# lambdaclass/simpleworks

Measured on AMD Instinct MI355X. Metric: Marlin prove() constraints/sec at 2^20 R1CS; G1 MSM points/sec, higher is better.
Workload: dtype u32 limbs (384-bit Montgomery Fq for G1, 256-bit Fr); 1 GPU; marlin_prove: synthetic R1CS, 2^20 constraints = variables = non-zeros per matrix (|H| = |K| = 2^20), SRS + proving key device resident; per_gpu_units=1048576, multi_gpu=replicas (one proof per rank)

## Files before the change

### simpleworks_amd/_lib.py

```python
import ctypes
import json
import os

import numpy as np

_HERE = os.path.dirname(os.path.abspath(__file__))
LIB_PATH = os.environ.get("SWM_LIB_PATH") or os.path.join(_HERE, "libswmarlin.so")

_u64p = ctypes.POINTER(ctypes.c_uint64)
_u32p = ctypes.POINTER(ctypes.c_uint32)
_vp = ctypes.c_void_p
_sz = ctypes.c_size_t
_int = ctypes.c_int

ABI = {
    "swm_version": (_int, []),
    "swm_strerror": (ctypes.c_char_p, [_int]),
    "swm_init": (_int, [_int, ctypes.POINTER(_vp)]),
    "swm_destroy": (None, [_vp]),
    "swm_last_error": (ctypes.c_char_p, [_vp]),
    "swm_set_stream": (_int, [_vp, _vp]),
    "swm_set_msm_sharding": (_int, [_vp, ctypes.c_uint, ctypes.c_uint, _vp, _vp]),
    "swm_rccl_unique_id": (_int, [ctypes.c_void_p]),
    "swm_rccl_init": (_int, [_vp, ctypes.c_void_p, ctypes.c_uint, ctypes.c_uint]),
# ... 431 lines not shown
        return out

    def selftest_poly_eval_many(self, buf_mont, pieces, z_mont):
        buf = np.ascontiguousarray(buf_mont, dtype=np.uint64).reshape(-1, 4)
        pc = np.asarray(pieces, dtype=np.uint64).reshape(-1, 2)
        out = np.zeros((pc.shape[0], 4), dtype=np.uint64)
        self._poly(3, buf, buf.shape[0], 0, z_mont, pc, out)
        return out

    def selftest_ntt_from(self, src_mont, log_n, inverse=False, coset=False):
        src = np.ascontiguousarray(src_mont, dtype=np.uint64).reshape(-1, 4).copy()
        out = np.zeros((1 << log_n, 4), dtype=np.uint64)
        self._poly(4 + int(bool(inverse)) + 2 * int(bool(coset)), src, src.shape[0], log_n, None, None, out)
        return out, src

    def selftest_scan(self, words):
        w = np.ascontiguousarray(words, dtype=np.uint32).reshape(-1)
        out = np.zeros(w.size + 1, dtype=np.uint32)
        self._poly(8, w, w.size, 0, None, None, out)
        return out[:-1], int(out[-1])

    def selftest_sample_fr(self, rng, need):
        out = np.zeros((max(need, 1), 4), dtype=np.uint64)
        self._check(self.lib.swm_selftest_sample_fr(self.h, rng.h, need, _p64(out)), "swm_selftest_sample_fr")
        return out[:need]

    def selftest_mul_throughput(self, which, threads, iters):
        ms = ctypes.c_float(0)
        self._check(self.lib.swm_selftest_mul_throughput(self.h, which, threads, iters, ctypes.byref(ms)),
                    "swm_selftest_mul_throughput")
# ... 2 lines not shown
```

### simpleworks_amd/csrc/devops.cuh

```cuda
#pragma once
#include <chrono>
#include <exception>
#include <functional>
#include <utility>
#include <atomic>
#include "context.h"
#include "ff.cuh"
#include "fill.cuh"
#include "fr29.cuh"
#include "host/chacha.h"
#include "host/marlin_types.h"

namespace swm {

int ntt_run(swm_ctx* ctx, void* d_data, unsigned log_n, int inverse, int coset);
int ntt_run_from(swm_ctx* ctx, void* d_data, unsigned log_n, int inverse, int coset, const void* first_src, size_t src_len);
int ntt_sharded_run(swm_ctx* ctx, void* d_local, unsigned log_n, int inverse, int blocks_in);
struct SpmvPlanHost {
    uint64_t nnz = 0, max_row = 0;
    std::vector<uint32_t> chunks, lrows;
};
struct SpmvPlan {
    uint64_t nnz = 0, max_row = 0;
    const uint32_t* d_chunks = nullptr;
    const uint32_t* d_lrows = nullptr;
    uint32_t n_chunks = 0, n_lrows = 0;
};
void spmv_plan_build(const uint32_t* rowptr, size_t rows, SpmvPlanHost* plan);
int spmv_run(swm_ctx* ctx, const void* d_rowptr, const void* d_col, const void* d_val, const void* d_z, void* d_out,
             size_t rows, const SpmvPlan* plan = nullptr);
int batch_inverse_run(swm_ctx* ctx, void* d, size_t n);
// ... 847 lines not shown
```

### simpleworks_amd/csrc/marlin.hip

```cpp
#include <stdlib.h>
#include <string.h>
#include <unistd.h>
#include <algorithm>
#include <chrono>
#include <functional>
#include <memory>
#include "devops.cuh"
#include "g1.cuh"
#include "host/ahp.h"

#include "msm.h"
using namespace swm;

#define LAUNCHX(ctx, name, kernel, grid, block, shmem, ...)                         \
    do {                                                                            \
        prof_begin(ctx, name);                                                      \
        hipLaunchKernelGGL(kernel, grid, block, shmem, (ctx)->stream, __VA_ARGS__); \
        prof_end(ctx);                                                              \
        hip_check(ctx, hipGetLastError(), name);                                    \
    } while (0)

#include "host/pk_codec.h"
#include "host/host_handles.h"
struct swm_srs {
// ... 1012 lines not shown
    ew(ctx, "div_vh", 3 * part, [=] __device__(size_t j) {
        Fr acc = q[j + part];
        if (j + 2 * part < total) acc = fp_add(acc, q[j + 2 * part]);
        if (j + 3 * part < total) acc = fp_add(acc, q[j + 3 * part]);
        h[j] = acc;
        if (j < part) g[j] = fp_add(q[j], acc);
    });
}
void div_vk(swm_ctx* ctx, const Fr* q, size_t part, size_t total, Fr* h) {
    ew(ctx, "div_vk", 3 * part, [=] __device__(size_t j) {
        Fr acc = fp_zero<Fr>();
        for (uint64_t i = 1; j + i * part < total; i++) acc = fp_add(acc, q[j + i * part]);
        h[j] = acc;
    });
}
struct RAlphaNumerators {
    Fr n0, n1, n2, n3;
};
RAlphaNumerators r_alpha_numerators(const Fr& alpha, unsigned logH, uint64_t M) {
    Fr aH = alpha;
    for (unsigned i = 0; i < logH; i++) aH = fp_sqr(aH);
    Fr i4 = HDomain(M).gen;
    for (unsigned i = 0; i < logH; i++) i4 = fp_sqr(i4);
    return {fp_sub(aH, fp_one<Fr>()), fp_sub(aH, i4), fp_sub(aH, fp_sqr(i4)), fp_sub(aH, fp_mul(fp_sqr(i4), i4))};
}
struct IndexOnB {
    const Fr *ar, *ac, *arc, *av;
    const Fr *br, *bc, *brc, *bv;
    const Fr *cr, *cc, *crc, *cv;
};
// ... 24 lines not shown
    const std::vector<Fr> public_input;
    FiatShamirRng fs;
    VerifierState st;
    Fr rho_w, rho_a, rho_b;
    int lane = 0;
    LPoly P_w, P_za, P_zb, P_mask, P_t, P_g1, P_h1, P_g2, P_h2;
    LPoly idx_polys[12];
    std::map<std::string, LPoly*> polys;
    CommitJob j1[4], j2[3], j3[2];
    std::vector<Commitment> comms1 = std::vector<Commitment>(4), comms2 = std::vector<Commitment>(3),
                            comms3 = std::vector<Commitment>(2);
    bool mask_late = false;
    unsigned mask_pieces = 1;
    AsyncMsm mask_part[2];
    bool ra_closed_form = false;
    LcSet lcs;
    DVec mask, z, za_evals, zb_evals, za_loc, zb_loc, x_poly, x_evals, w_poly, za_poly, zb_poly, e_za, e_zb, e_z;
    DVec r_alpha_evals, e_ra, t_poly, q1, h1, g1x, f, h2;

    ProveState(const swm_pk& pk, ChaChaRng& rng, PhaseTrace& t, ProveShape shp, const ShardPlan& plan)
        : zk(rng), tr(t), shape(std::move(shp)), sp(plan), H(pk.H), K(pk.K), X(pk.X), Bsz(pk.B), M(4 * pk.H),
          logM(pk.logH + 2), nvars(pk.info.num_variables), ninst(shape.inst.size()), mask_len(3 * pk.H), dh(pk.H),
          public_input(shape.inst.begin() + 1, shape.inst.end()) {
        fs_init(fs, pk.vk, public_input);
        for (int m = 0; m < 3; m++) {
            const DVec* v[4] = {&pk.ar[m].row, &pk.ar[m].col, &pk.ar[m].val, &pk.ar[m].row_col};
            for (int j = 0; j < 4; j++) {
                idx_polys[4 * m + j].p = v[j]->p;
                idx_polys[4 * m + j].n = K;
                polys[kIndexerPolys[4 * m + j]] = &idx_polys[4 * m + j];
// ... 155 lines not shown
        sharded_interpolate_and_commit(ctx, pk, s, s.zb_loc, s.rho_b, s.zb_poly, &s.j1[2]);
    } else {
        rc_check(ctx, ntt_run_from(ctx, s.za_poly.p, pk.logH, 1, 0, s.za_evals.p, H));
        add_rho_vh(ctx, s.za_poly.p, H, s.rho_a);
        rc_check(ctx, ntt_run_from(ctx, s.zb_poly.p, pk.logH, 1, 0, s.zb_evals.p, H));
        add_rho_vh(ctx, s.zb_poly.p, H, s.rho_b);
        pc_commit_begin(ctx, pk, &s.lane, s.P_za.p, s.P_za.n, false, 0, true, &s.j1[1]);
        pc_commit_begin(ctx, pk, &s.lane, s.P_zb.p, s.P_zb.n, false, 0, true, &s.j1[2]);
    }
}

DVec on_mul_domain(swm_ctx* ctx, const ProveState& s, const Fr* coeffs, size_t n) {
    if (!s.sp.r2) return dv_ntt_from(ctx, coeffs, n, s.logM, false);
    return shard_evals(ctx, s.sp, coeffs, n, s.logM);
}
void round2_prework(swm_ctx* ctx, ProveState& s) {
    const uint64_t H = s.H, X = s.X;
    s.e_za = on_mul_domain(ctx, s, s.za_poly.p, H + 1);
    s.e_zb = on_mul_domain(ctx, s, s.zb_poly.p, H + 1);
    DVec z_poly = dv_zeros(ctx, H + 1);
    Fr* out = z_poly.p;
    const Fr* wc = s.P_w.p;
    const size_t w_len = s.P_w.n;
    const Fr* xp = s.x_poly.p;
    ew(ctx, "z_poly", H + 1, [=] __device__(size_t i) {
        Fr v = fp_zero<Fr>();
        if (i >= X && i - X < w_len) v = wc[i - X];
        if (i < w_len) v = fp_sub(v, wc[i]);
        if (i < X) v = fp_add(v, xp[i]);
        out[i] = v;
    });
    s.e_z = on_mul_domain(ctx, s, z_poly.p, H + 1);
}

void round1_commitments(swm_ctx* ctx, const swm_pk& pk, ProveState& s) {
    pc_commit_blind(pk, &s.j1[0], &s.zk, &s.P_w.rand);
    pc_commit_blind(pk, &s.j1[1], &s.zk, &s.P_za.rand);
    pc_commit_blind(pk, &s.j1[2], &s.zk, &s.P_zb.rand);
    pc_commit_blind(pk, &s.j1[3], nullptr, &s.P_mask.rand);
    if (s.mask_pieces > 1) {
        Fr c0 = s.mask.download(0, 1)[0];
        Fr c0s = fp_to_std(c0);
        G1XYZZ extra = g1_mul_limbs(pk.vk.vk.g, c0s.v, 8);
        for (unsigned k = 0; k + 1 < s.mask_pieces; k++) g1_add(extra, commit_wait(ctx, &s.mask_part[k]));
        s.j1[3].has_extra = true;
        s.j1[3].extra = extra;
    }
// ... 26 lines not shown
        s.e_ra = DVec(ctx, mloc);
        PowTable wt = root_pow_table(ctx, s.logM);
        Fr* out = s.e_ra.p;
        ew(ctx, "r_alpha_den", mloc, [=] __device__(size_t p) {
            const size_t i = mloc * (p / mblk) + s_rank * mblk + (p % mblk);
            out[p] = fp_sub(alpha, wt.at(i));
        });
        rc_check(ctx, batch_inverse_run(ctx, out, mloc));
        const RAlphaNumerators nu = r_alpha_numerators(alpha, pk.logH, M);
        ew(ctx, "r_alpha_scale", mloc, [=] __device__(size_t p) {
            const size_t i = mloc * (p / mblk) + s_rank * mblk + (p % mblk);
            const unsigned q = (unsigned)(i & 3);
            out[p] = fp_mul(out[p], q == 0 ? nu.n0 : q == 1 ? nu.n1 : q == 2 ? nu.n2 : nu.n3);
        });
        r_alpha_on_h(ctx, pk, s);
    } else {
        s.e_ra = DVec(ctx, M);
        PowTable wt = root_pow_table(ctx, s.logM);
        Fr* out = s.e_ra.p;
        ew(ctx, "r_alpha_den", M, [=] __device__(size_t i) { out[i] = fp_sub(alpha, wt.at(i)); });
        rc_check(ctx, batch_inverse_run(ctx, out, M));
        const RAlphaNumerators nu = r_alpha_numerators(alpha, pk.logH, M);
        Fr* rh = s.r_alpha_evals.p;
        ew(ctx, "r_alpha_scale", M, [=] __device__(size_t i) {
            const unsigned q = (unsigned)(i & 3);
            Fr v = fp_mul(out[i], q == 0 ? nu.n0 : q == 1 ? nu.n1 : q == 2 ? nu.n2 : nu.n3);
            out[i] = v;
            if (q == 0) rh[i >> 2] = v;
        });
    }
// ... 4 lines not shown
    const size_t nvars = s.nvars;
    const Fr eta_a = s.st.eta_a, eta_b = s.st.eta_b, eta_c = s.st.eta_c;
    s.t_poly = dv_zeros(ctx, H);
    {
        DVec ta(ctx, nvars), tb(ctx, nvars), tc(ctx, nvars);
        const Fr* ra = s.r_alpha_evals.p;
        rc_check(ctx, spmv_run(ctx, pk.at.rowptr.p, pk.at.col.p, pk.at.val.p, ra, ta.p, nvars, &pk.at.plan));
        rc_check(ctx, spmv_run(ctx, pk.bt.rowptr.p, pk.bt.col.p, pk.bt.val.p, ra, tb.p, nvars, &pk.bt.plan));
        rc_check(ctx, spmv_run(ctx, pk.ct.rowptr.p, pk.ct.col.p, pk.ct.val.p, ra, tc.p, nvars, &pk.ct.plan));
        Fr* out = s.t_poly.p;
        const Fr *pa = ta.p, *pb = tb.p, *pc = tc.p;
        ew(ctx, "t_evals", nvars, [=] __device__(size_t c) {
            Fr v = fp_add(fp_add(fp_mul(eta_a, pa[c]), fp_mul(eta_b, pb[c])), fp_mul(eta_c, pc[c]));
            out[reindex_by_subdomain(H, X, c)] = v;
        });
        dv_ntt(ctx, s.t_poly, pk.logH, true);
    }
    s.tr.tick("r2: t polynomial enqueued");
    s.P_t.p = s.t_poly.p;
    s.P_t.n = H;
    pc_commit_begin(ctx, pk, &s.lane, s.P_t.p, s.P_t.n, false, 0, false, &s.j2[0]);
}

void round2_q1(swm_ctx* ctx, const swm_pk& pk, ProveState& s) {
    const uint64_t H = s.H, M = s.M;
    const size_t Mloc = s.sp.Mloc;
    const Fr eta_a = s.st.eta_a, eta_b = s.st.eta_b, eta_c = s.st.eta_c;
    s.q1 = DVec(ctx, Mloc);
    {
        if (!s.ra_closed_form) {
            DVec ra_poly = dv_ntt_from(ctx, s.r_alpha_evals.p, H, pk.logH, true);
            s.e_ra = on_mul_domain(ctx, s, ra_poly.p, H);
        }
        DVec e_t = on_mul_domain(ctx, s, s.t_poly.p, H);
        Fr* out = s.q1.p;
        const Fr *pra = s.e_ra.p, *pza = s.e_za.p, *pzb = s.e_zb.p, *pt = e_t.p, *pz = s.e_z.p;
        ew(ctx, "round2_pointwise", Mloc, [=] __device__(size_t i) {
            Fr a = pza[i], b = pzb[i];
            Fr summed = fp_add(fp_add(fp_mul(eta_c, fp_mul(a, b)), fp_mul(eta_a, a)), fp_mul(eta_b, b));
// ... 47 lines not shown
    pc_commit_blind(pk, &s.j2[1], &s.zk, &s.P_g1.rand);
    pc_commit_blind(pk, &s.j2[2], nullptr, &s.P_h1.rand);
    commit_gather(ctx, {&s.j2[0].plain, &s.j2[1].plain, &s.j2[1].shifted, &s.j2[2].plain});
    pc_commit_end_round(ctx, pk, {&s.j2[0], &s.j2[1], &s.j2[2]}, {nullptr, &s.zk, nullptr},
                        {&s.P_t.rand, &s.P_g1.rand, &s.P_h1.rand}, s.comms2.data());
    if (unsat && !ctx->emulated_exchange)
        throw MarlinError(SWM_ERR_UNSATISFIED, "outer sumcheck does not hold: constraint system is not satisfied");
}

void round3_polys(swm_ctx* ctx, const swm_pk& pk, ProveState& s) {
    const uint64_t K = s.K, Bsz = s.Bsz;
    const Fr alpha = s.st.alpha, beta = s.st.beta;
    const Fr eta_a = s.st.eta_a, eta_b = s.st.eta_b, eta_c = s.st.eta_c;
    const Fr vhab = fp_mul(s.dh.vanishing(alpha), s.dh.vanishing(beta));
    s.f = DVec(ctx, K);
    {
        DVec inv(ctx, 3 * K);
        for (int m = 0; m < 3; m++) {
            Fr* out = inv.p + (size_t)m * K;
            const Fr *rk = pk.ar[m].row_K.p, *ck = pk.ar[m].col_K.p;
            ew(ctx, "round3_den_K", K, [=] __device__(size_t i) { out[i] = fp_mul(fp_sub(beta, rk[i]), fp_sub(alpha, ck[i])); });
        }
        rc_check(ctx, batch_inverse_run(ctx, inv.p, 3 * K));
        Fr* out = s.f.p;
        const Fr *ia = inv.p, *ib = inv.p + K, *ic = inv.p + 2 * K;
        const Fr *va = pk.ar[0].val_K.p, *vb = pk.ar[1].val_K.p, *vc = pk.ar[2].val_K.p;
        ew(ctx, "round3_f_K", K, [=] __device__(size_t i) {
            Fr t = fp_add(fp_add(fp_mul(fp_mul(eta_a, va[i]), ia[i]), fp_mul(fp_mul(eta_b, vb[i]), ib[i])),
                          fp_mul(fp_mul(eta_c, vc[i]), ic[i]));
            out[i] = fp_mul(vhab, t);
        });
        dv_ntt(ctx, s.f, pk.logK, true);
    }
    s.P_g2.p = s.f.p + 1; s.P_g2.n = K - 1; s.P_g2.has_bound = true; s.P_g2.bound = K - 2;
    pc_commit_begin(ctx, pk, &s.lane, s.P_g2.p, s.P_g2.n, true, K - 2, false, &s.j3[0]);
    s.h2 = DVec(ctx, 3 * K);
    const IndexOnB ix{pk.ar[0].row_B.p, pk.ar[0].col_B.p, pk.ar[0].row_col_B.p, pk.ar[0].val_B.p,
                      pk.ar[1].row_B.p, pk.ar[1].col_B.p, pk.ar[1].row_col_B.p, pk.ar[1].val_B.p,
                      pk.ar[2].row_B.p, pk.ar[2].col_B.p, pk.ar[2].row_col_B.p, pk.ar[2].val_B.p};
    const Round3Challenges ch{alpha, beta, fp_mul(beta, alpha), eta_a, eta_b, eta_c, vhab};
    if (s.sp.r3) {
        const size_t Bloc = Bsz / s.sp.SG, Bblk = Bloc / s.sp.SG, Kl = K / s.sp.SG, s_rank = s.sp.rank;
        DVec e_f = shard_evals(ctx, s.sp, s.f.p, K, pk.logB);
        DVec ab(ctx, Bloc);
        Fr* out = ab.p;
        const Fr* pf = e_f.p;
        ew(ctx, "round3_pointwise_B", Bloc, [=] __device__(size_t p) {
            const size_t i = Bloc * (p / Bblk) + s_rank * Bblk + (p % Bblk);
            out[p] = round3_a_minus_bf(ix, ch, i, pf[p]);
        });
        rc_check(ctx, ntt_sharded_run(ctx, ab.p, pk.logB, 1, 1));
        DVec loc(ctx, 3 * Kl);
        div_vk(ctx, ab.p, Kl, Bloc, loc.p);
        shard_gather_cyclic(ctx, loc.p, 3 * Kl, s.sp.slog_g, s.h2.p, 3 * K);
    } else {
        DVec e_f = dv_ntt_from(ctx, s.f.p, K, pk.logB, false);
        DVec ab(ctx, Bsz);
        Fr* out = ab.p;
        const Fr* pf = e_f.p;
        ew(ctx, "round3_pointwise_B", Bsz, [=] __device__(size_t i) { out[i] = round3_a_minus_bf(ix, ch, i, pf[i]); });
        dv_ntt(ctx, ab, pk.logB, true);
        div_vk(ctx, ab.p, K, Bsz, s.h2.p);
    }
    s.P_h2.p = s.h2.p;
    s.P_h2.n = 3 * K >= 3 ? 3 * K - 3 : 0;
}

std::vector<Fr> evaluations(swm_ctx* ctx, const swm_pk& pk, ProveState& s) {
    std::map<std::pair<std::string, bool>, Fr> eval_cache;
// ... 688 lines not shown
static void selftest_poly_impl(swm_ctx* ctx, int op, void* data, size_t n, size_t m, const uint64_t* z, const uint64_t* pieces,
                               size_t npieces, void* out) {
    Fr zz = fp_zero<Fr>();
    if (z) memcpy(zz.v, z, 32);
    if (op == 8) {
        DBuf<uint32_t> in(ctx, n), res(ctx, n);
        if (n) in.upload((const uint32_t*)data, n);
        const uint32_t total = scan_exclusive_u32(ctx, in.p, res.p, n);
        std::vector<uint32_t> h = res.download(0, n);
        if (n) memcpy(out, h.data(), n * 4);
        ((uint32_t*)out)[n] = total;
        return;
    }
    DVec a(ctx, n);
    if (n) a.upload((const Fr*)data, n);
    if (op == 0) {
        suffix_recurrence(ctx, a.p, n, m, zz);
        std::vector<Fr> h = a.download(0, n);
        if (n) memcpy(data, h.data(), n * sizeof(Fr));
    } else if (op == 1) {
        DivResult r = div_linear(ctx, a.p, n, zz);
        std::vector<Fr> h = r.work.download(0, n);
        if (n) memcpy(out, h.data(), n * sizeof(Fr));
    } else if (op == 2) {
        const Fr v = poly_eval(ctx, a.p, n, zz);
        memcpy(out, v.v, sizeof(Fr));
    } else if (op == 3) {
        for (size_t i = 0; i < npieces; i++)
            if (pieces[2 * i] > n || pieces[2 * i + 1] > n - pieces[2 * i]) throw MarlinError(SWM_ERR_INVALID_ARG, "piece out of range");
        DVec res(ctx, npieces);
// ... 1 lines not shown
        for (size_t i = 0; i < npieces; i++) items.push_back({a.p + pieces[2 * i], (size_t)pieces[2 * i + 1], res.p + i});
        EvalPoint ep = eval_point(ctx, zz);
        poly_eval_many(ctx, items, ep);
        std::vector<Fr> h = res.download(0, npieces);
        if (npieces) memcpy(out, h.data(), npieces * sizeof(Fr));
    } else {
        DVec t = dv_ntt_from(ctx, a.p, n, (unsigned)m, ((op - 4) & 1) != 0, ((op - 4) & 2) != 0);
        std::vector<Fr> h = t.download(0, t.n);
        memcpy(out, h.data(), t.n * sizeof(Fr));
        std::vector<Fr> s = a.download(0, n);
        if (n) memcpy(data, s.data(), n * sizeof(Fr));
    }
}
int swm_selftest_poly(swm_ctx* ctx, int op, void* data, size_t n, size_t m, const uint64_t z[4], const uint64_t* pieces,
                      size_t npieces, void* out) {
    if (!ctx || op < 0 || op > 8 || (n && !data)) return SWM_ERR_INVALID_ARG;
    if ((op >= 1 && op <= 3 && !z) || (op == 0 && (!z || m == 0)) || (op != 0 && !out) || (op == 3 && npieces && !pieces))
        return SWM_ERR_INVALID_ARG;
    if (op >= 4 && op <= 7 && (m < 1 || m > 28 || n > ((size_t)1 << m))) return SWM_ERR_INVALID_ARG;
    SWM_ON_DEVICE(ctx);
    SWM_GUARD(ctx, selftest_poly_impl(ctx, op, data, n, m, z, pieces, npieces, out));
}
static void selftest_sample_impl(swm_ctx* ctx, ChaChaRng& rng, size_t need, uint64_t* out_mont) {
    DVec d(ctx, need);
    sample_fr_bulk(ctx, rng, d.p, need);
    std::vector<Fr> h = d.download(0, need);
    if (need) memcpy(out_mont, h.data(), need * sizeof(Fr));
}
int swm_selftest_sample_fr(swm_ctx* ctx, swm_rng* rng, size_t need, uint64_t* out_mont) {
    if (!ctx || !rng || (need && !out_mont)) return SWM_ERR_INVALID_ARG;
    SWM_ON_DEVICE(ctx);
    SWM_GUARD(ctx, selftest_sample_impl(ctx, rng->r, need, out_mont));
}

// ... 41 lines not shown
```

### simpleworks_amd/csrc/ntt.hip

```cpp
#include <atomic>
#include "context.h"
#include "ff.cuh"
#include "fr29.cuh"
#include <string.h>
#include <algorithm>
#include <vector>

namespace swm {

static constexpr int NTT_THREADS = 256;
static constexpr unsigned NTT_MAX_LOG_R = 10;

struct NttPassArgs {
    const Fr* src;
    Fr* dst;
    unsigned log_n, log_r, log_ns;
    const Fr* tw_small;
    const Fr* tw_lo;
    const Fr* tw_hi;
    const Fr* cs_lo;
    const Fr* cs_hi;
    uint64_t src_len;
    const Fr* pass_tw;
    int coset_in;
    int scale_out;
    int coset_out;
    Fr n_inv;
};

__device__ __forceinline__ Fr two_level_pow(const Fr* lo, const Fr* hi, uint64_t e) {
    Fr a = lo[e & 1023];
    uint64_t h = e >> 10;
    if (h) a = fp_mul(a, hi[h]);
    return a;
}

__device__ __forceinline__ unsigned bitrev_u(unsigned x, unsigned bits) { return bits ? (__brev(x) >> (32 - bits)) : 0u; }

template <int J>
__global__ void __launch_bounds__(NTT_THREADS) ntt_pass(NttPassArgs a) {
    SWM_LIGHT_KERNEL();
    extern __shared__ __align__(16) unsigned char smem_raw[];
    Fr* tile = reinterpret_cast<Fr*>(smem_raw);
    const unsigned R = 1u << a.log_r;
    const uint64_t n = 1ull << a.log_n;
    const uint64_t stride = n >> a.log_r;
    const uint64_t j0 = (uint64_t)blockIdx.x * J;
    const uint64_t ns_mask = (1ull << a.log_ns) - 1;
    const unsigned tw_shift = a.log_n - a.log_ns - a.log_r;
    for (unsigned e0 = 0; e0 < R * J; e0 += 4 * NTT_THREADS) {
        Fr xs[4];
#pragma unroll
        for (int u = 0; u < 4; u++) {
            unsigned e = e0 + threadIdx.x + u * NTT_THREADS;
            if (e < R * J) {
                const uint64_t at = j0 + e % J + (uint64_t)(e / J) * stride;
                xs[u] = at < a.src_len ? a.src[at] : fp_zero<Fr>();
            }
        }
#pragma unroll
        for (int u = 0; u < 4; u++) {
            unsigned e = e0 + threadIdx.x + u * NTT_THREADS;
            if (e >= R * J) break;
            unsigned jj = e % J, t = e / J;
            uint64_t idx = j0 + jj + (uint64_t)t * stride;
            Fr x = xs[u];
            if (a.coset_in) x = fp_mul(x, two_level_pow(a.cs_lo, a.cs_hi, idx));
            if (a.log_ns != 0 && t != 0) {
                uint64_t k = (j0 + jj) & ns_mask;
                if (k) x = fp_mul(x, two_level_pow(a.tw_lo, a.tw_hi, (k * t) << tw_shift));
            }
            tile[t * J + jj] = x;
        }
    }
    __syncthreads();
    unsigned h = R >> 1;
    if (a.log_r & 1) {
        for (unsigned bq = threadIdx.x; bq < (R >> 1) * J; bq += NTT_THREADS) {
            unsigned jj = bq % J, pos = bq / J;
            unsigned i0 = pos, i1 = i0 + h;
            Fr u = tile[i0 * J + jj], v = tile[i1 * J + jj];
            tile[i0 * J + jj] = fp_add(u, v);
// ... 30 lines not shown
    for (unsigned e = threadIdx.x; e < R * J; e += NTT_THREADS) {
        unsigned jj, u;
        if (a.log_ns == 0) {
            u = e % R;
            jj = e / R;
        } else {
            jj = e % J;
            u = e / J;
        }
        uint64_t j = j0 + jj;
        uint64_t k = j & ns_mask;
        uint64_t o = ((j - k) << a.log_r) + k + ((uint64_t)u << a.log_ns);
        Fr x = tile[bitrev_u(u, a.log_r) * J + jj];
        if (a.scale_out) {
            Fr s = a.n_inv;
            if (a.coset_out) s = fp_mul(s, two_level_pow(a.cs_lo, a.cs_hi, o));
            x = fp_mul(x, s);
        }
        a.dst[o] = x;
    }
}

struct LazyPlan {
    Spread29 r2;
    Spread29 s1[6];
    Spread29 s2[6];
    Spread29 s4;
    uint32_t reduce;
    uint32_t out_below_2r;
};
struct NttLazyArgs {
    NttPassArgs a;
    LazyPlan plan;
    int last_pass;
// ... 18 lines not shown
    return x;
}
template <int J>
__global__ void __launch_bounds__(NTT_THREADS, 4) ntt_pass_lazy(NttLazyArgs args) {
    SWM_LIGHT_KERNEL();
    extern __shared__ __align__(16) unsigned char smem_raw[];
    uint32_t* tile = reinterpret_cast<uint32_t*>(smem_raw);
    const NttPassArgs& a = args.a;
    const LazyPlan& P = args.plan;
    const unsigned R = 1u << a.log_r;
    const uint64_t n = 1ull << a.log_n;
    const uint64_t stride = n >> a.log_r;
    const uint64_t j0 = (uint64_t)blockIdx.x * J;
    const uint64_t ns_mask = (1ull << a.log_ns) - 1;
    const unsigned tw_shift = a.log_n - a.log_ns - a.log_r;
    for (unsigned e0 = 0; e0 < R * J; e0 += 4 * NTT_THREADS) {
        Fr xs[4];
#pragma unroll
        for (int u = 0; u < 4; u++) {
            unsigned e = e0 + threadIdx.x + u * NTT_THREADS;
            if (e < R * J) {
                const uint64_t at = j0 + e % J + (uint64_t)(e / J) * stride;
                xs[u] = at < a.src_len ? a.src[at] : fp_zero<Fr>();
            }
        }
#pragma unroll
        for (int u = 0; u < 4; u++) {
            unsigned e = e0 + threadIdx.x + u * NTT_THREADS;
            if (e >= R * J) break;
            unsigned jj = e % J, t = e / J;
            uint64_t idx = j0 + jj + (uint64_t)t * stride;
            Fr29 x = fr29_unpack(xs[u]);
            if (a.coset_in) x = fr29_mul_fenced(x, two_level_pow29(a.cs_lo, a.cs_hi, idx));
            if (a.log_ns != 0) {
                uint64_t k = (j0 + jj) & ns_mask;
                const Fr29 tw = a.pass_tw ? fr29_unpack(a.pass_tw[((uint64_t)t << a.log_ns) + k])
                                          : two_level_pow29(a.tw_lo, a.tw_hi, (k * t) << tw_shift);
                x = fr29_mul_fenced(x, tw);
            }
            tile_put(tile, t * J + jj, x);
        }
    }
    __syncthreads();
    unsigned h = R >> 1;
    if (a.log_r & 1) {
        for (unsigned bq = threadIdx.x; bq < (R >> 1) * J; bq += NTT_THREADS) {
            unsigned jj = bq % J, pos = bq / J;
            unsigned i0 = pos, i1 = i0 + h;
// ... 38 lines not shown
    for (unsigned e = threadIdx.x; e < R * J; e += NTT_THREADS) {
        unsigned jj, u;
        if (a.log_ns == 0) {
            u = e % R;
            jj = e / R;
        } else {
            jj = e % J;
            u = e / J;
        }
        uint64_t j = j0 + jj;
        uint64_t k = j & ns_mask;
        uint64_t o = ((j - k) << a.log_r) + k + ((uint64_t)u << a.log_ns);
        Fr29 x = tile_get(tile, bitrev_u(u, a.log_r) * J + jj);
        if (a.scale_out) {
            Fr29 sc = fr29_unpack(a.n_inv);
            if (a.coset_out) sc = fr29_mul_fenced(two_level_pow29(a.cs_lo, a.cs_hi, o), sc);
            x = fr29_canonical(fr29_mul_fenced(x, sc), true);
        } else if (args.last_pass) {
            x = fr29_canonical(x, P.out_below_2r != 0);
        }
        a.dst[o] = fr29_pack(x);
    }
}

static Fr host_root_of_unity(unsigned log_n, bool inverse) {
    Fr w;
    const uint32_t root[8] = SWM_FR_ROOT47_MONT;
    for (int i = 0; i < 8; i++) w.v[i] = root[i];
    for (unsigned i = log_n; i < 47; i++) w = fp_sqr(w);
    if (inverse) w = fp_inv(w);
    return w;
}

static int upload_powers(swm_ctx* ctx, const Fr& base, size_t count, void** out, bool lazy29 = false) {
    std::vector<Fr> h(count);
    Fr cur = lazy29 ? fp_from_u64<Fr>(32) : fp_one<Fr>();
// ... 124 lines not shown
        P.s1[st] = lazy_spread(2 * B, 1);
        P.s2[st] = lazy_spread(4 * B, 2);
        const bool red = 4 * B > 64 || st + 1 == nsteps;
        if (red) P.reduce |= 1u << st;
        B = red ? 4 : 4 * B;
    }
    P.s4 = lazy_spread(4, 1);
    P.out_below_2r = B <= 2 ? 1u : 0u;
    return P;
}

int ntt_run_from(swm_ctx* ctx, void* d_data, unsigned log_n, int inverse, int coset, const void* first_src, size_t src_len);
int ntt_run(swm_ctx* ctx, void* d_data, unsigned log_n, int inverse, int coset) {
    return ntt_run_from(ctx, d_data, log_n, inverse, coset, nullptr, 0);
}
int ntt_run_from(swm_ctx* ctx, void* d_data, unsigned log_n, int inverse, int coset, const void* first_src, size_t src_len) {
    if (log_n > 30) return set_err(ctx, SWM_ERR_INVALID_ARG, "ntt: log_n > 30 unsupported");
    const uint64_t n = 1ull << log_n;
    if (first_src && src_len > n) src_len = n;
    ctx->stat_ntt_calls++;
    ctx->log_call('n', log_n);
    ctx->stat_ntt_elems += n;
    Fr* data = reinterpret_cast<Fr*>(d_data);
    const unsigned maxr = NTT_MAX_LOG_R;
    static const bool lazy = env_switch("SWM_NTT_LAZY", 1, 0, 1) != 0;
    NttTables *rt = nullptr, *ct = nullptr;
    SWM_TRY(get_root_tables_form(ctx, log_n, inverse, lazy, &rt));
    if (coset) SWM_TRY(get_coset_tables(ctx, log_n, inverse, &ct, lazy));
    Fr n_inv = fp_one<Fr>();
    if (inverse) n_inv = fp_inv(fp_from_u64<Fr>(n));
    if (lazy) n_inv = fp_mul(n_inv, fp_from_u64<Fr>(32));
    unsigned npass = log_n <= maxr ? 1 : (log_n + maxr - 1) / maxr;
    unsigned radices[8];
    {
        unsigned rem = log_n;
        for (unsigned p = 0; p < npass; p++) {
            unsigned r = (rem + (npass - p) - 1) / (npass - p);
            radices[p] = r;
            rem -= r;
        }
    }
    Fr *tmp = nullptr, *tmp2 = nullptr;
    SWM_TRY(scratch(ctx, "ntt.tmp", n * sizeof(Fr), (void**)&tmp));
    if (npass % 2 == 1 && npass >= 3) SWM_TRY(scratch(ctx, "ntt.tmp2", n * sizeof(Fr), (void**)&tmp2));
    const Fr* src = first_src ? reinterpret_cast<const Fr*>(first_src) : data;
    if (npass == 1 && !first_src) {
        SWM_HIP(ctx, hipMemcpyAsync(tmp, data, n * sizeof(Fr), hipMemcpyDeviceToDevice, ctx->stream));
        src = tmp;
    }
    unsigned log_ns = 0;
    for (unsigned p = 0; p < npass; p++) {
        NttPassArgs a;
        a.src = src;
        if (p == npass - 1) a.dst = data;
        else if (tmp2) a.dst = (p % 2 == 0) ? tmp : tmp2;
        else a.dst = (src == tmp) ? data : tmp;
        a.src_len = (p == 0 && first_src) ? (uint64_t)src_len : n;
        a.log_n = log_n;
        a.log_r = radices[p];
        a.log_ns = log_ns;
        SWM_TRY(get_small_table(ctx, a.log_r, inverse, &a.tw_small, lazy));
        a.tw_lo = reinterpret_cast<const Fr*>(rt->lo);
        a.tw_hi = reinterpret_cast<const Fr*>(rt->hi);
        a.cs_lo = ct ? reinterpret_cast<const Fr*>(ct->lo) : nullptr;
        a.cs_hi = ct ? reinterpret_cast<const Fr*>(ct->hi) : nullptr;
        a.pass_tw = nullptr;
        if (lazy && log_ns != 0) SWM_TRY(get_pass_table(ctx, log_n, inverse, log_ns, a.log_r, rt, &a.pass_tw));
        a.coset_in = (coset && !inverse && p == 0) ? 1 : 0;
        a.scale_out = (inverse && p == npass - 1) ? 1 : 0;
        a.coset_out = (coset && inverse && p == npass - 1) ? 1 : 0;
        a.n_inv = n_inv;
        uint64_t cols = n >> a.log_r;
        if (lazy) {
            NttLazyArgs la;
            la.a = a;
            la.plan = lazy_plan(a.log_r, (p > 0 || a.coset_in) ? 2u : 1u);
            la.last_pass = p == npass - 1 ? 1 : 0;
            unsigned J = 1;
            if (npass > 1) {
                J = (log_n >= 19 ? 1024u : 512u) >> a.log_r;
                if (J < 1) J = 1;
                if (J > 16) J = 16;
                while (J > cols) J >>= 1;
            }
            const size_t elems = (size_t)J << a.log_r;
            size_t shmem = (elems + (elems >> 5) + 1) * 36;
            if (shmem < 64) shmem = 64;
            dim3 grid((unsigned)(cols / J)), block(NTT_THREADS);
            if (shmem > 64 * 1024) {
                static std::atomic<size_t> granted[64];
                if (J != 1 || shmem > 160 * 1024) return set_err(ctx, SWM_ERR_INVALID_ARG, "ntt: tile does not fit LDS");
                if (granted[ctx->device & 63].load() < shmem) {
                    SWM_HIP(ctx, hipFuncSetAttribute((const void*)ntt_pass_lazy<1>, hipFuncAttributeMaxDynamicSharedMemorySize, (int)shmem));
                    granted[ctx->device & 63].store(shmem);
                }
            }
            switch (J) {
                case 1: SWM_LAUNCH(ctx, "ntt_pass", ntt_pass_lazy<1>, grid, block, shmem, la); break;
                case 2: SWM_LAUNCH(ctx, "ntt_pass", ntt_pass_lazy<2>, grid, block, shmem, la); break;
                case 4: SWM_LAUNCH(ctx, "ntt_pass", ntt_pass_lazy<4>, grid, block, shmem, la); break;
                case 8: SWM_LAUNCH(ctx, "ntt_pass", ntt_pass_lazy<8>, grid, block, shmem, la); break;
                default: SWM_LAUNCH(ctx, "ntt_pass", ntt_pass_lazy<16>, grid, block, shmem, la); break;
            }
        } else if (npass == 1) {
            size_t shmem = sizeof(Fr) << a.log_r;
            if (shmem < 64) shmem = 64;
            SWM_LAUNCH(ctx, "ntt_pass", ntt_pass<1>, dim3((unsigned)cols), dim3(NTT_THREADS), shmem, a);
        } else {
            unsigned J = (log_n >= 19 ? 1024u : 512u) >> a.log_r;
            if (J < 1) J = 1;
            if (J > 16) J = 16;
            while (J > cols) J >>= 1;
            size_t shmem = (sizeof(Fr) * J) << a.log_r;
            dim3 grid((unsigned)(cols / J)), block(NTT_THREADS);
            switch (J) {
                case 1: SWM_LAUNCH(ctx, "ntt_pass", ntt_pass<1>, grid, block, shmem, a); break;
                case 2: SWM_LAUNCH(ctx, "ntt_pass", ntt_pass<2>, grid, block, shmem, a); break;
                case 4: SWM_LAUNCH(ctx, "ntt_pass", ntt_pass<4>, grid, block, shmem, a); break;
                case 8: SWM_LAUNCH(ctx, "ntt_pass", ntt_pass<8>, grid, block, shmem, a); break;
                default: SWM_LAUNCH(ctx, "ntt_pass", ntt_pass<16>, grid, block, shmem, a); break;
            }
        }
        log_ns += a.log_r;
        src = a.dst;
    }
    return SWM_OK;
}


// ... 72 lines not shown
```

Baseline: 22.04 million constraints/s.

## Evaluate Marlin round-2/3 quotients on size-H cosets instead of 4H domain

Round 2 now evaluates z_A, z_B, z and t on two cosets of H (plus the H domain itself) rather than running full 4H-size NTTs. Round 2 also does an inverse NTT per coset and recovers the three H-sized pieces with a small closed-form solve that uses the 4th root of unity and 1/2. Round 3 reuses the already-known evaluations of f on K and only transforms the three remaining cosets. Multi-coset NTTs are batched through blockIdx.y, with coset twiddles and folding of inputs longer than n done inside the pass kernels. The aim is to cut NTT size and memory traffic at the cost of added kernel-argument complexity and a new code path restricted to non-sharded runs.

```diff
diff --git a/simpleworks_amd/_lib.py b/simpleworks_amd/_lib.py
--- a/simpleworks_amd/_lib.py
+++ b/simpleworks_amd/_lib.py
@@ -469,6 +469,20 @@
         self._poly(4 + int(bool(inverse)) + 2 * int(bool(coset)), src, src.shape[0], log_n, None, None, out)
         return out, src
 
+    def selftest_ntt_cosets(self, coeffs_mont, log_n, ks):
+        src = np.ascontiguousarray(coeffs_mont, dtype=np.uint64).reshape(-1, 4).copy()
+        kk = np.ascontiguousarray(ks, dtype=np.uint64).reshape(-1)
+        out = np.zeros((kk.size << log_n, 4), dtype=np.uint64)
+        self._check(self.lib.swm_selftest_poly(self.h, 9, src.ctypes.data, src.shape[0], log_n, _p64(np.zeros(4, np.uint64)),
+                                               _p64(kk), kk.size, out.ctypes.data), "swm_selftest_poly")
+        return out.reshape(kk.size, 1 << log_n, 4)
+
+    def selftest_intt_cosets3(self, evals_mont, log_n):
+        ev = np.ascontiguousarray(evals_mont, dtype=np.uint64).reshape(-1, 4).copy()
+        out = np.zeros_like(ev)
+        self._poly(10, ev, ev.shape[0], log_n, None, None, out)
+        return out
+
     def selftest_scan(self, words):
         w = np.ascontiguousarray(words, dtype=np.uint32).reshape(-1)
         out = np.zeros(w.size + 1, dtype=np.uint32)
diff --git a/simpleworks_amd/csrc/devops.cuh b/simpleworks_amd/csrc/devops.cuh
--- a/simpleworks_amd/csrc/devops.cuh
+++ b/simpleworks_amd/csrc/devops.cuh
@@ -15,6 +15,8 @@
 
 int ntt_run(swm_ctx* ctx, void* d_data, unsigned log_n, int inverse, int coset);
 int ntt_run_from(swm_ctx* ctx, void* d_data, unsigned log_n, int inverse, int coset, const void* first_src, size_t src_len);
+int ntt_cosets_fwd(swm_ctx* ctx, const void* coeffs, size_t len, unsigned log_n, const unsigned* ks, unsigned ncos, void* out);
+int ntt_cosets_inv(swm_ctx* ctx, void* data, unsigned log_n, unsigned ncos);
 int ntt_sharded_run(swm_ctx* ctx, void* d_local, unsigned log_n, int inverse, int blocks_in);
 struct SpmvPlanHost {
     uint64_t nnz = 0, max_row = 0;
diff --git a/simpleworks_amd/csrc/marlin.hip b/simpleworks_amd/csrc/marlin.hip
--- a/simpleworks_amd/csrc/marlin.hip
+++ b/simpleworks_amd/csrc/marlin.hip
@@ -1050,6 +1050,20 @@
         h[j] = acc;
     });
 }
+#ifndef SWM_OUTER_COSETS
+#define SWM_OUTER_COSETS 1
+#endif
+static constexpr uint64_t OUTER_COSETS_MIN_H = 16;
+struct Cosets3 {
+    Fr p0, p1, p2;
+};
+__device__ __forceinline__ Cosets3 cosets3_solve(const Fr& u0, const Fr& u1, const Fr& u2, const Fr& iota, const Fr& half) {
+    const Fr p1 = fp_mul(fp_sub(u0, u2), half);
+    const Fr e = fp_mul(fp_add(u0, u2), half);
+    const Fr d = fp_sub(u1, fp_mul(iota, p1));
+    return {fp_mul(fp_add(e, d), half), p1, fp_mul(fp_sub(e, d), half)};
+}
+static Fr fr_half() { return fp_inv(fp_from_u64<Fr>(2)); }
 struct RAlphaNumerators {
     Fr n0, n1, n2, n3;
 };
@@ -1104,6 +1118,7 @@
     unsigned mask_pieces = 1;
     AsyncMsm mask_part[2];
     bool ra_closed_form = false;
+    bool cosets = false;
     LcSet lcs;
     DVec mask, z, za_evals, zb_evals, za_loc, zb_loc, x_poly, x_evals, w_poly, za_poly, zb_poly, e_za, e_zb, e_z;
     DVec r_alpha_evals, e_ra, t_poly, q1, h1, g1x, f, h2;
@@ -1289,10 +1304,19 @@
     if (!s.sp.r2) return dv_ntt_from(ctx, coeffs, n, s.logM, false);
     return shard_evals(ctx, s.sp, coeffs, n, s.logM);
 }
+DVec on_cosets12(swm_ctx* ctx, const ProveState& s, const Fr* coeffs, size_t n) {
+    static const unsigned ks[2] = {1, 2};
+    DVec v(ctx, 2 * s.H);
+    rc_check(ctx, ntt_cosets_fwd(ctx, coeffs, n, s.dh.log, ks, 2, v.p));
+    return v;
+}
 void round2_prework(swm_ctx* ctx, ProveState& s) {
     const uint64_t H = s.H, X = s.X;
-    s.e_za = on_mul_domain(ctx, s, s.za_poly.p, H + 1);
-    s.e_zb = on_mul_domain(ctx, s, s.zb_poly.p, H + 1);
+    s.cosets = SWM_OUTER_COSETS && !s.sp.r1 && !s.sp.r2 && H >= OUTER_COSETS_MIN_H && s.mask_len == 3 * H &&
+               !env_flag("SWM_RALPHA_TRANSFORMS");
+    auto on_domain = [&](const Fr* coeffs, size_t n) { return s.cosets ? on_cosets12(ctx, s, coeffs, n) : on_mul_domain(ctx, s, coeffs, n); };
+    s.e_za = on_domain(s.za_poly.p, H + 1);
+    s.e_zb = on_domain(s.zb_poly.p, H + 1);
     DVec z_poly = dv_zeros(ctx, H + 1);
     Fr* out = z_poly.p;
     const Fr* wc = s.P_w.p;
@@ -1305,7 +1329,7 @@
         if (i < X) v = fp_add(v, xp[i]);
         out[i] = v;
     });
-    s.e_z = on_mul_domain(ctx, s, z_poly.p, H + 1);
+    s.e_z = on_domain(z_poly.p, H + 1);
 }
 
 void round1_commitments(swm_ctx* ctx, const swm_pk& pk, ProveState& s) {
@@ -1362,6 +1386,22 @@
             out[p] = fp_mul(out[p], q == 0 ? nu.n0 : q == 1 ? nu.n1 : q == 2 ? nu.n2 : nu.n3);
         });
         r_alpha_on_h(ctx, pk, s);
+    } else if (s.cosets) {
+        const uint64_t H = s.H;
+        const unsigned logH = pk.logH;
+        s.e_ra = DVec(ctx, 3 * H);
+        PowTable wt = root_pow_table(ctx, s.logM);
+        Fr* out = s.e_ra.p;
+        ew(ctx, "r_alpha_den", 3 * H, [=] __device__(size_t p) { out[p] = fp_sub(alpha, wt.at(((p & (H - 1)) << 2) + (p >> logH))); });
+        rc_check(ctx, batch_inverse_run(ctx, out, 3 * H));
+        const RAlphaNumerators nu = r_alpha_numerators(alpha, pk.logH, M);
+        Fr* rh = s.r_alpha_evals.p;
+        ew(ctx, "r_alpha_scale", 3 * H, [=] __device__(size_t p) {
+            const size_t q = p >> logH;
+            Fr v = fp_mul(out[p], q == 0 ? nu.n0 : q == 1 ? nu.n1 : nu.n2);
+            out[p] = v;
+            if (q == 0) rh[p] = v;
+        });
     } else {
         s.e_ra = DVec(ctx, M);
         PowTable wt = root_pow_table(ctx, s.logM);
@@ -1396,6 +1436,23 @@
             Fr v = fp_add(fp_add(fp_mul(eta_a, pa[c]), fp_mul(eta_b, pb[c])), fp_mul(eta_c, pc[c]));
             out[reindex_by_subdomain(H, X, c)] = v;
         });
+        if (s.cosets) {
+            s.q1 = DVec(ctx, 3 * H);
+            Fr* q = s.q1.p;
+            const Fr *rh = s.r_alpha_evals.p, *za = s.za_evals.p, *zb = s.zb_evals.p, *th = s.t_poly.p, *zz = s.z.p, *xe = s.x_evals.p;
+            const uint64_t ratio = H / X;
+            const size_t nwit = s.shape.nwit, ninst = s.ninst;
+            ew(ctx, "round2_pointwise_h", H, [=] __device__(size_t k) {
+                Fr zk = xe[k];
+                if (k % ratio != 0) {
+                    const size_t wi = k - k / ratio - 1;
+                    zk = wi < nwit ? zz[ninst + wi] : fp_zero<Fr>();
+                }
+                const Fr a = za[k], b = zb[k];
+                const Fr summed = fp_add(fp_add(fp_mul(eta_c, fp_mul(a, b)), fp_mul(eta_a, a)), fp_mul(eta_b, b));
+                q[k] = fp_sub(fp_mul(rh[k], summed), fp_mul(zk, th[k]));
+            });
+        }
         dv_ntt(ctx, s.t_poly, pk.logH, true);
     }
     s.tr.tick("r2: t polynomial enqueued");
@@ -1404,7 +1461,47 @@
     pc_commit_begin(ctx, pk, &s.lane, s.P_t.p, s.P_t.n, false, 0, false, &s.j2[0]);
 }
 
+void round2_q1_cosets(swm_ctx* ctx, const swm_pk& pk, ProveState& s) {
+    const uint64_t H = s.H;
+    const Fr eta_a = s.st.eta_a, eta_b = s.st.eta_b, eta_c = s.st.eta_c;
+    if (!s.ra_closed_form) {
+        DVec ra_poly = dv_ntt_from(ctx, s.r_alpha_evals.p, H, pk.logH, true);
+        DVec e12 = on_cosets12(ctx, s, ra_poly.p, H);
+        s.e_ra = DVec(ctx, 3 * H);
+        hip_check(ctx, hipMemcpyAsync(s.e_ra.p + H, e12.p, 2 * H * sizeof(Fr), hipMemcpyDeviceToDevice, ctx->stream), "copy");
+    }
+    {
+        DVec e_t = on_cosets12(ctx, s, s.t_poly.p, H);
+        Fr* out = s.q1.p + H;
+        const Fr *pra = s.e_ra.p + H, *pza = s.e_za.p, *pzb = s.e_zb.p, *pt = e_t.p, *pz = s.e_z.p;
+        ew(ctx, "round2_pointwise", 2 * H, [=] __device__(size_t i) {
+            Fr a = pza[i], b = pzb[i];
+            Fr summed = fp_add(fp_add(fp_mul(eta_c, fp_mul(a, b)), fp_mul(eta_a, a)), fp_mul(eta_b, b));
+            out[i] = fp_sub(fp_mul(pra[i], summed), fp_mul(pz[i], pt[i]));
+        });
+        s.e_za.release();
+        s.e_zb.release();
+        s.e_z.release();
+    }
+    rc_check(ctx, ntt_cosets_inv(ctx, s.q1.p, pk.logH, 3));
+    s.h1 = DVec(ctx, 3 * H);
+    s.g1x = DVec(ctx, H);
+    const Fr* q = s.q1.p;
+    const Fr* mp = s.mask.p;
+    Fr *h = s.h1.p, *g = s.g1x.p;
+    const Fr iota = HDomain(4).gen, half = fr_half();
+    ew(ctx, "q1_cosets_solve_div_vh", H, [=] __device__(size_t j) {
+        const Cosets3 c = cosets3_solve(q[j], q[j + H], q[j + 2 * H], iota, half);
+        const Fr p0 = fp_add(c.p0, mp[j]), p1 = fp_add(c.p1, mp[j + H]), p2 = fp_add(c.p2, mp[j + 2 * H]);
+        const Fr hj = fp_add(p1, p2);
+        h[j] = hj;
+        h[j + H] = p2;
+        h[j + 2 * H] = fp_zero<Fr>();
+        g[j] = fp_add(p0, hj);
+    });
+}
 void round2_q1(swm_ctx* ctx, const swm_pk& pk, ProveState& s) {
+    if (s.cosets) return round2_q1_cosets(ctx, pk, s);
     const uint64_t H = s.H, M = s.M;
     const size_t Mloc = s.sp.Mloc;
     const Fr eta_a = s.st.eta_a, eta_b = s.st.eta_b, eta_c = s.st.eta_c;
@@ -1482,6 +1579,8 @@
     const Fr eta_a = s.st.eta_a, eta_b = s.st.eta_b, eta_c = s.st.eta_c;
     const Fr vhab = fp_mul(s.dh.vanishing(alpha), s.dh.vanishing(beta));
     s.f = DVec(ctx, K);
+    const bool f_cosets = SWM_OUTER_COSETS && !s.sp.r3 && Bsz == 4 * K && K >= OUTER_COSETS_MIN_H;
+    DVec f_K;
     {
         DVec inv(ctx, 3 * K);
         for (int m = 0; m < 3; m++) {
@@ -1493,12 +1592,17 @@
         Fr* out = s.f.p;
         const Fr *ia = inv.p, *ib = inv.p + K, *ic = inv.p + 2 * K;
         const Fr *va = pk.ar[0].val_K.p, *vb = pk.ar[1].val_K.p, *vc = pk.ar[2].val_K.p;
+        if (f_cosets) {
+            f_K = DVec(ctx, K);
+            out = f_K.p;
+        }
         ew(ctx, "round3_f_K", K, [=] __device__(size_t i) {
             Fr t = fp_add(fp_add(fp_mul(fp_mul(eta_a, va[i]), ia[i]), fp_mul(fp_mul(eta_b, vb[i]), ib[i])),
                           fp_mul(fp_mul(eta_c, vc[i]), ic[i]));
             out[i] = fp_mul(vhab, t);
         });
-        dv_ntt(ctx, s.f, pk.logK, true);
+        if (f_cosets) rc_check(ctx, ntt_run_from(ctx, s.f.p, pk.logK, 1, 0, f_K.p, K));
+        else dv_ntt(ctx, s.f, pk.logK, true);
     }
     s.P_g2.p = s.f.p + 1; s.P_g2.n = K - 1; s.P_g2.has_bound = true; s.P_g2.bound = K - 2;
     pc_commit_begin(ctx, pk, &s.lane, s.P_g2.p, s.P_g2.n, true, K - 2, false, &s.j3[0]);
@@ -1521,6 +1625,20 @@
         DVec loc(ctx, 3 * Kl);
         div_vk(ctx, ab.p, Kl, Bloc, loc.p);
         shard_gather_cyclic(ctx, loc.p, 3 * Kl, s.sp.slog_g, s.h2.p, 3 * K);
+    } else if (f_cosets) {
+        static const unsigned ks[3] = {1, 2, 3};
+        DVec e_f(ctx, 3 * K);
+        rc_check(ctx, ntt_cosets_fwd(ctx, s.f.p, K, pk.logK, ks, 3, e_f.p));
+        DVec ab(ctx, Bsz);
+        Fr* out = ab.p;
+        const Fr *pf = e_f.p, *fk = f_K.p;
+        const unsigned logK = pk.logK;
+        ew(ctx, "round3_pointwise_B", Bsz, [=] __device__(size_t i) {
+            const size_t k = i & 3, j = i >> 2;
+            out[i] = round3_a_minus_bf(ix, ch, i, k ? pf[((k - 1) << logK) + j] : fk[j]);
+        });
+        dv_ntt(ctx, ab, pk.logB, true);
+        div_vk(ctx, ab.p, K, Bsz, s.h2.p);
     } else {
         DVec e_f = dv_ntt_from(ctx, s.f.p, K, pk.logB, false);
         DVec ab(ctx, Bsz);
@@ -2239,6 +2357,32 @@
     }
     DVec a(ctx, n);
     if (n) a.upload((const Fr*)data, n);
+    if (op == 9) {
+        unsigned ks[4];
+        for (size_t c = 0; c < npieces; c++) ks[c] = (unsigned)pieces[c];
+        DVec t(ctx, npieces << m);
+        rc_check(ctx, ntt_cosets_fwd(ctx, a.p, n, (unsigned)m, ks, (unsigned)npieces, t.p));
+        std::vector<Fr> h = t.download(0, t.n);
+        memcpy(out, h.data(), t.n * sizeof(Fr));
+        return;
+    }
+    if (op == 10) {
+        const size_t N = (size_t)1 << m;
+        rc_check(ctx, ntt_cosets_inv(ctx, a.p, (unsigned)m, 3));
+        DVec t(ctx, 3 * N);
+        const Fr* u = a.p;
+        Fr* o = t.p;
+        const Fr iota = HDomain(4).gen, half = fr_half();
+        ew(ctx, "cosets3_solve", N, [=] __device__(size_t j) {
+            const Cosets3 c = cosets3_solve(u[j], u[j + N], u[j + 2 * N], iota, half);
+            o[j] = c.p0;
+            o[j + N] = c.p1;
+            o[j + 2 * N] = c.p2;
+        });
+        std::vector<Fr> h = t.download(0, t.n);
+        memcpy(out, h.data(), t.n * sizeof(Fr));
+        return;
+    }
     if (op == 0) {
         suffix_recurrence(ctx, a.p, n, m, zz);
         std::vector<Fr> h = a.download(0, n);
@@ -2270,10 +2414,16 @@
 }
 int swm_selftest_poly(swm_ctx* ctx, int op, void* data, size_t n, size_t m, const uint64_t z[4], const uint64_t* pieces,
                       size_t npieces, void* out) {
-    if (!ctx || op < 0 || op > 8 || (n && !data)) return SWM_ERR_INVALID_ARG;
+    if (!ctx || op < 0 || op > 10 || (n && !data)) return SWM_ERR_INVALID_ARG;
     if ((op >= 1 && op <= 3 && !z) || (op == 0 && (!z || m == 0)) || (op != 0 && !out) || (op == 3 && npieces && !pieces))
         return SWM_ERR_INVALID_ARG;
     if (op >= 4 && op <= 7 && (m < 1 || m > 28 || n > ((size_t)1 << m))) return SWM_ERR_INVALID_ARG;
+    if (op == 9) {
+        if (m < 1 || m > 26 || n > ((size_t)2 << m) || npieces < 1 || npieces > 4 || !pieces) return SWM_ERR_INVALID_ARG;
+        for (size_t c = 0; c < npieces; c++)
+            if (pieces[c] > 3) return SWM_ERR_INVALID_ARG;
+    }
+    if (op == 10 && (m < 1 || m > 26 || n != ((size_t)3 << m))) return SWM_ERR_INVALID_ARG;
     SWM_ON_DEVICE(ctx);
     SWM_GUARD(ctx, selftest_poly_impl(ctx, op, data, n, m, z, pieces, npieces, out));
 }
diff --git a/simpleworks_amd/csrc/ntt.hip b/simpleworks_amd/csrc/ntt.hip
--- a/simpleworks_amd/csrc/ntt.hip
+++ b/simpleworks_amd/csrc/ntt.hip
@@ -26,6 +26,10 @@
     int scale_out;
     int coset_out;
     Fr n_inv;
+    uint64_t src_cstride, dst_cstride;
+    uint32_t cos_k[4];
+    int fold_in;
+    Fr fold[4];
 };
 
 __device__ __forceinline__ Fr two_level_pow(const Fr* lo, const Fr* hi, uint64_t e) {
@@ -48,6 +52,9 @@
     const uint64_t j0 = (uint64_t)blockIdx.x * J;
     const uint64_t ns_mask = (1ull << a.log_ns) - 1;
     const unsigned tw_shift = a.log_n - a.log_ns - a.log_r;
+    const Fr* src = a.src + blockIdx.y * a.src_cstride;
+    Fr* dst = a.dst + blockIdx.y * a.dst_cstride;
+    const uint64_t cs_k = a.cos_k[blockIdx.y];
     for (unsigned e0 = 0; e0 < R * J; e0 += 4 * NTT_THREADS) {
         Fr xs[4];
 #pragma unroll
@@ -55,7 +62,8 @@
             unsigned e = e0 + threadIdx.x + u * NTT_THREADS;
             if (e < R * J) {
                 const uint64_t at = j0 + e % J + (uint64_t)(e / J) * stride;
-                xs[u] = at < a.src_len ? a.src[at] : fp_zero<Fr>();
+                xs[u] = at < a.src_len ? src[at] : fp_zero<Fr>();
+                if (a.fold_in && at + n < a.src_len) xs[u] = fp_add(xs[u], fp_mul(a.fold[blockIdx.y], src[at + n]));
             }
         }
 #pragma unroll
@@ -65,7 +73,7 @@
             unsigned jj = e % J, t = e / J;
             uint64_t idx = j0 + jj + (uint64_t)t * stride;
             Fr x = xs[u];
-            if (a.coset_in) x = fp_mul(x, two_level_pow(a.cs_lo, a.cs_hi, idx));
+            if (a.coset_in) x = fp_mul(x, two_level_pow(a.cs_lo, a.cs_hi, idx * cs_k));
             if (a.log_ns != 0 && t != 0) {
                 uint64_t k = (j0 + jj) & ns_mask;
                 if (k) x = fp_mul(x, two_level_pow(a.tw_lo, a.tw_hi, (k * t) << tw_shift));
@@ -126,10 +134,10 @@
         Fr x = tile[bitrev_u(u, a.log_r) * J + jj];
         if (a.scale_out) {
             Fr s = a.n_inv;
-            if (a.coset_out) s = fp_mul(s, two_level_pow(a.cs_lo, a.cs_hi, o));
+            if (a.coset_out) s = fp_mul(s, two_level_pow(a.cs_lo, a.cs_hi, o * cs_k));
             x = fp_mul(x, s);
         }
-        a.dst[o] = x;
+        dst[o] = x;
     }
 }
 
@@ -178,6 +186,9 @@
     const uint64_t j0 = (uint64_t)blockIdx.x * J;
     const uint64_t ns_mask = (1ull << a.log_ns) - 1;
     const unsigned tw_shift = a.log_n - a.log_ns - a.log_r;
+    const Fr* src = a.src + blockIdx.y * a.src_cstride;
+    Fr* dst = a.dst + blockIdx.y * a.dst_cstride;
+    const uint64_t cs_k = a.cos_k[blockIdx.y];
     for (unsigned e0 = 0; e0 < R * J; e0 += 4 * NTT_THREADS) {
         Fr xs[4];
 #pragma unroll
@@ -185,7 +196,8 @@
             unsigned e = e0 + threadIdx.x + u * NTT_THREADS;
             if (e < R * J) {
                 const uint64_t at = j0 + e % J + (uint64_t)(e / J) * stride;
-                xs[u] = at < a.src_len ? a.src[at] : fp_zero<Fr>();
+                xs[u] = at < a.src_len ? src[at] : fp_zero<Fr>();
+                if (a.fold_in && at + n < a.src_len) xs[u] = fp_add(xs[u], fp_mul(a.fold[blockIdx.y], src[at + n]));
             }
         }
 #pragma unroll
@@ -195,7 +207,7 @@
             unsigned jj = e % J, t = e / J;
             uint64_t idx = j0 + jj + (uint64_t)t * stride;
             Fr29 x = fr29_unpack(xs[u]);
-            if (a.coset_in) x = fr29_mul_fenced(x, two_level_pow29(a.cs_lo, a.cs_hi, idx));
+            if (a.coset_in) x = fr29_mul_fenced(x, two_level_pow29(a.cs_lo, a.cs_hi, idx * cs_k));
             if (a.log_ns != 0) {
                 uint64_t k = (j0 + jj) & ns_mask;
                 const Fr29 tw = a.pass_tw ? fr29_unpack(a.pass_tw[((uint64_t)t << a.log_ns) + k])
@@ -264,12 +276,12 @@
         Fr29 x = tile_get(tile, bitrev_u(u, a.log_r) * J + jj);
         if (a.scale_out) {
             Fr29 sc = fr29_unpack(a.n_inv);
-            if (a.coset_out) sc = fr29_mul_fenced(two_level_pow29(a.cs_lo, a.cs_hi, o), sc);
+            if (a.coset_out) sc = fr29_mul_fenced(two_level_pow29(a.cs_lo, a.cs_hi, o * cs_k), sc);
             x = fr29_canonical(fr29_mul_fenced(x, sc), true);
         } else if (args.last_pass) {
             x = fr29_canonical(x, P.out_below_2r != 0);
         }
-        a.dst[o] = fr29_pack(x);
+        dst[o] = fr29_pack(x);
     }
 }
 
@@ -424,19 +436,46 @@
 int ntt_run(swm_ctx* ctx, void* d_data, unsigned log_n, int inverse, int coset) {
     return ntt_run_from(ctx, d_data, log_n, inverse, coset, nullptr, 0);
 }
+static int ntt_run_multi(swm_ctx* ctx, void* d_data, unsigned log_n, int inverse, int coset, const void* first_src, size_t src_len,
+                         unsigned ncos, const unsigned* ks);
 int ntt_run_from(swm_ctx* ctx, void* d_data, unsigned log_n, int inverse, int coset, const void* first_src, size_t src_len) {
+    if (first_src && src_len > (1ull << std::min(log_n, 62u))) src_len = 1ull << log_n;
+    return ntt_run_multi(ctx, d_data, log_n, inverse, coset ? 1 : 0, first_src, src_len, 1, nullptr);
+}
+int ntt_cosets_fwd(swm_ctx* ctx, const void* coeffs, size_t len, unsigned log_n, const unsigned* ks, unsigned ncos, void* out) {
+    if (ncos < 1 || ncos > 4 || log_n > 28 || len > (2ull << log_n)) return set_err(ctx, SWM_ERR_INVALID_ARG, "ntt cosets: bad shape");
+    for (unsigned c = 0; c < ncos; c++)
+        if (ks[c] > 3) return set_err(ctx, SWM_ERR_INVALID_ARG, "ntt cosets: coset index > 3");
+    return ntt_run_multi(ctx, out, log_n, 0, 2, coeffs, len, ncos, ks);
+}
+int ntt_cosets_inv(swm_ctx* ctx, void* data, unsigned log_n, unsigned ncos) {
+    if (ncos < 1 || ncos > 4 || log_n > 28) return set_err(ctx, SWM_ERR_INVALID_ARG, "ntt cosets: bad shape");
+    const unsigned ks[4] = {0, 1, 2, 3};
+    return ntt_run_multi(ctx, data, log_n, 1, 2, nullptr, 0, ncos, ks);
+}
+static int ntt_run_multi(swm_ctx* ctx, void* d_data, unsigned log_n, int inverse, int coset, const void* first_src, size_t src_len,
+                         unsigned ncos, const unsigned* ks) {
     if (log_n > 30) return set_err(ctx, SWM_ERR_INVALID_ARG, "ntt: log_n > 30 unsupported");
     const uint64_t n = 1ull << log_n;
-    if (first_src && src_len > n) src_len = n;
-    ctx->stat_ntt_calls++;
-    ctx->log_call('n', log_n);
-    ctx->stat_ntt_elems += n;
+    for (unsigned c = 0; c < ncos; c++) {
+        ctx->stat_ntt_calls++;
+        ctx->log_call('n', log_n);
+        ctx->stat_ntt_elems += n;
+    }
     Fr* data = reinterpret_cast<Fr*>(d_data);
+    const uint64_t total = n * ncos;
     const unsigned maxr = NTT_MAX_LOG_R;
     static const bool lazy = env_switch("SWM_NTT_LAZY", 1, 0, 1) != 0;
     NttTables *rt = nullptr, *ct = nullptr;
     SWM_TRY(get_root_tables_form(ctx, log_n, inverse, lazy, &rt));
-    if (coset) SWM_TRY(get_coset_tables(ctx, log_n, inverse, &ct, lazy));
+    if (coset == 1) SWM_TRY(get_coset_tables(ctx, log_n, inverse, &ct, lazy));
+    if (coset == 2) SWM_TRY(get_root_tables_form(ctx, log_n + 2, inverse, lazy, &ct));
+    Fr fold[4];
+    for (unsigned c = 0; c < 4; c++) {
+        fold[c] = fp_one<Fr>();
+        if (coset == 2 && c < ncos)
+            for (unsigned e = 0; e < ks[c]; e++) fold[c] = fp_mul(fold[c], host_root_of_unity(2, false));
+    }
     Fr n_inv = fp_one<Fr>();
     if (inverse) n_inv = fp_inv(fp_from_u64<Fr>(n));
     if (lazy) n_inv = fp_mul(n_inv, fp_from_u64<Fr>(32));
@@ -451,11 +490,11 @@
         }
     }
     Fr *tmp = nullptr, *tmp2 = nullptr;
-    SWM_TRY(scratch(ctx, "ntt.tmp", n * sizeof(Fr), (void**)&tmp));
-    if (npass % 2 == 1 && npass >= 3) SWM_TRY(scratch(ctx, "ntt.tmp2", n * sizeof(Fr), (void**)&tmp2));
+    SWM_TRY(scratch(ctx, "ntt.tmp", total * sizeof(Fr), (void**)&tmp));
+    if (npass % 2 == 1 && npass >= 3) SWM_TRY(scratch(ctx, "ntt.tmp2", total * sizeof(Fr), (void**)&tmp2));
     const Fr* src = first_src ? reinterpret_cast<const Fr*>(first_src) : data;
     if (npass == 1 && !first_src) {
-        SWM_HIP(ctx, hipMemcpyAsync(tmp, data, n * sizeof(Fr), hipMemcpyDeviceToDevice, ctx->stream));
+        SWM_HIP(ctx, hipMemcpyAsync(tmp, data, total * sizeof(Fr), hipMemcpyDeviceToDevice, ctx->stream));
         src = tmp;
     }
     unsigned log_ns = 0;
@@ -480,6 +519,13 @@
         a.scale_out = (inverse && p == npass - 1) ? 1 : 0;
         a.coset_out = (coset && inverse && p == npass - 1) ? 1 : 0;
         a.n_inv = n_inv;
+        a.src_cstride = (p == 0 && first_src) ? 0 : n;
+        a.dst_cstride = n;
+        a.fold_in = (coset == 2 && a.coset_in && src_len > n) ? 1 : 0;
+        for (unsigned c = 0; c < 4; c++) {
+            a.cos_k[c] = coset == 2 ? (c < ncos ? ks[c] : 0) : 1;
+            a.fold[c] = fold[c];
+        }
         uint64_t cols = n >> a.log_r;
         if (lazy) {
             NttLazyArgs la;
@@ -496,7 +542,7 @@
             const size_t elems = (size_t)J << a.log_r;
             size_t shmem = (elems + (elems >> 5) + 1) * 36;
             if (shmem < 64) shmem = 64;
-            dim3 grid((unsigned)(cols / J)), block(NTT_THREADS);
+            dim3 grid((unsigned)(cols / J), ncos), block(NTT_THREADS);
             if (shmem > 64 * 1024) {
                 static std::atomic<size_t> granted[64];
                 if (J != 1 || shmem > 160 * 1024) return set_err(ctx, SWM_ERR_INVALID_ARG, "ntt: tile does not fit LDS");
@@ -515,14 +561,14 @@
         } else if (npass == 1) {
             size_t shmem = sizeof(Fr) << a.log_r;
             if (shmem < 64) shmem = 64;
-            SWM_LAUNCH(ctx, "ntt_pass", ntt_pass<1>, dim3((unsigned)cols), dim3(NTT_THREADS), shmem, a);
+            SWM_LAUNCH(ctx, "ntt_pass", ntt_pass<1>, dim3((unsigned)cols, ncos), dim3(NTT_THREADS), shmem, a);
         } else {
             unsigned J = (log_n >= 19 ? 1024u : 512u) >> a.log_r;
             if (J < 1) J = 1;
             if (J > 16) J = 16;
             while (J > cols) J >>= 1;
             size_t shmem = (sizeof(Fr) * J) << a.log_r;
-            dim3 grid((unsigned)(cols / J)), block(NTT_THREADS);
+            dim3 grid((unsigned)(cols / J), ncos), block(NTT_THREADS);
             switch (J) {
                 case 1: SWM_LAUNCH(ctx, "ntt_pass", ntt_pass<1>, grid, block, shmem, a); break;
                 case 2: SWM_LAUNCH(ctx, "ntt_pass", ntt_pass<2>, grid, block, shmem, a); break;
```

New measurement: 22.52 million constraints/s, median of 6. 1.02x the previous value.
